# rimelq/VISTAF-RoboSkin-Vision-Integrated-Multimodal-Sensor

Hardware: AMD Instinct MI355X
Metric: frames/sec (224x224 -> force-map) at batch 256 (higher is better)
Workload: dtype f32; 1 GPU; BASELINE configs[2]: batch 256/GPU of 224x224x3 fp16 fringe frames (256 distinct frames) -> 224x224 f32 depth map + force scalars, full FTP path (inpaint, demod, unwrap, detrend, compose, force tail), constants scaled-224; inputs resident in HBM; global_batch=256, input_dtype=fp16, constants=scaled, parallelism=dp1, inflight_batches=3, frames_with_nonzero_status=0

## Files before the change

vistaf-roboskin-vision-integrated-multimodal-sensor_amd/_lib.py:

```python
from __future__ import annotations

import ctypes
import os

_HERE = os.path.dirname(os.path.abspath(__file__))
LIB_PATH = os.path.join(_HERE, "libvistaf_ftp.so")

NSCALARS = 16
NREFINFO = 8
NCONTACT = 16
MAX_CONTACTS = 64
NTRACK = 16
TRACK_NAMES = ["track_id", "age_frames", "parent_row", "events", "overlap_px", "dx", "dy", "dforce_N", "dvolume_cm3", "origin_track_id"]
TRACK_EVENTS = {"born": 1, "split": 2, "merged": 4, "gated": 8}
FATE_ENDED, FATE_NO_ROW = -1, -2 ** 31
NSHAPE = 24
SHAPE_NAMES = ["contact_pixels", "boundary_pixels", "footprint_cx", "footprint_cy", "major_axis_mm", "minor_axis_mm", "orientation_rad",
               "fit_pixels", "fit_status", "apex_x", "apex_y", "apex_depth_mm", "curvature_1_per_mm", "curvature_2_per_mm",
               "curvature_axis_rad", "radius_1_mm", "radius_2_mm", "fit_rms_mm"]
SHAPE_FIT = {"ok": 0, "none": 1, "not_a_cap": 2}
NTAXEL, NTAXELFRAME, TAXEL_NONE = 12, 8, 0xFFFF
TAXEL_NAMES = ["contact_pixels", "contact_area_mm2", "volume_cm3", "mean_depth_mm", "max_depth_mm", "argmax_index", "centroid_x", "centroid_y",
               "force_N", "pressure_kPa"]
TAXEL_FRAME_NAMES = ["active_taxels", "volume_cm3", "force_N", "cop_x", "cop_y", "moment_x_Nmm", "moment_y_Nmm", "peak_taxel"]
# ... 239 lines not shown
MASK_CHAIN_SIGNATURES = {
    "vistaf_ftp_test_mask_chain_fits": (ci, [ci, ci, ci, ci, ci, ci]),
    "vistaf_ftp_test_bad_chain": (ci, [vp, vp, vp, vp, vp, ci, ci, vp, vp, ci, ci, ci, ci, vp]),
    "vistaf_ftp_test_reliable_chain": (ci, [vp, vp, vp, ci, ci, ci, vp, vp, vp, vp, ci, ci, ci, ci, vp]),
    "vistaf_ftp_test_contact_chain": (ci, [vp, vp, vp, vp, cd, cd, ci, ci, vp, vp, vp, vp, ci, ci, ci, ci, vp]),
}
DFT_STAGED_SIGNATURES = {
    "vistaf_ftp_test_dft_forward_v": (ci, [vp, vp, vp, vp, sz, sz, vp, ci, vp, vp, ci, ci, ci, ci, ci, ci, ci, vp]),
    "vistaf_ftp_test_dft_inverse_v": (ci, [vp, ci, vp, vp, sz, sz, vp, vp, vp, vp, vp, sz, vp, vp, vp, ci, ci, ci, ci, ci, ci, vp]),
    "vistaf_ftp_test_dft_staged_fits": (ci, [ci, ci, ci, ci, ci]),
}
GAUSS_STRIP_SIGNATURES = {
    "vistaf_ftp_test_gauss_variant": (ci, [vp, vp, cd, ci, ci, ci, ci, vp]),
    "vistaf_ftp_test_gauss_strip_fits": (ci, [ci, ci, ci]),
}
OUTLINE_SIGNATURES = {
    "vistaf_outline_workspace_bytes": (ci, [ci, ci, ci, ci, P(sz)]),
    "vistaf_outline_measure": (ci, [vp, vp, vp, vp, ci, ci, ci, ci, ci, vp, vp, vp, vp, sz, vp]),
}
TEXTURE_SIGNATURES = {
    "vistaf_texture_workspace_bytes": (ci, [ci, ci, ci, ci, ci, P(sz)]),
    "vistaf_texture_measure": (ci, [vp, vp, vp, vp, vp, cf, cd, ci, ci, cd, cd, ci, ci, ci, ci, vp, vp, vp, vp, sz, vp]),
}
MATCH_SIGNATURES = {
    "vistaf_match_bank_bytes": (ci, [ci, ci, ci, P(i32), P(sz)]),
    "vistaf_match_build_bank": (ci, [P(cf), P(i32), P(i32), ci, ci, ci, cd, vp, sz]),
    "vistaf_match_workspace_bytes": (ci, [ci, ci, ci, ci, ci, ci, ci, P(sz)]),
    "vistaf_match_measure": (ci, [vp, vp, vp, vp, vp, vp, sz, P(i32), cf, ci, ci, cd, cd, ci, ci, ci, ci, vp, vp, vp, vp, sz, vp]),
}
CENTRELINE_SIGNATURES = {
# ... 7 lines not shown
 TEMPORAL_EXPORTS, CLOUD_EXPORTS, MOTION_EXPORTS, PRESSURE_EXPORTS) = (list(group) for group in SIGNATURES.values())

_lib = None


def load():
    global _lib
    if _lib is not None:
        return _lib
    if not os.path.exists(LIB_PATH):
        raise RuntimeError(
            f"{LIB_PATH} is missing: build it with `python __graft_entry__.py` (hipcc --offload-arch=gfx950). "
            "This package has no CPU path."
        )
    lib = ctypes.CDLL(LIB_PATH)
    for group in list(SIGNATURES.values()) + [MASK_CHAIN_SIGNATURES, DFT_STAGED_SIGNATURES, GAUSS_STRIP_SIGNATURES, OUTLINE_SIGNATURES, TEXTURE_SIGNATURES, MATCH_SIGNATURES,
                                                 CENTRELINE_SIGNATURES, CENTRELINE_TEST_SIGNATURES]:
        for name, (restype, argtypes) in group.items():
            fn = getattr(lib, name)
            fn.restype, fn.argtypes = restype, argtypes
    _lib = lib
    return lib


def check(rc: int):
    if rc != 0:
        msg = load().vistaf_ftp_last_error().decode("utf-8", "replace")
        if rc == -1:
            raise ValueError(msg)
        raise RuntimeError(f"vistaf_ftp error {rc}: {msg}")
```

vistaf-roboskin-vision-integrated-multimodal-sensor_amd/csrc/api.hip:

```cpp
#include <hip/hip_runtime.h>
#include <algorithm>
#include <cmath>
#include <cstdio>
#include <cstdlib>
#include <cstring>
#include <map>
#include <string>
#include <vector>

#include "host_util.hpp"
#include "mask_rules.hpp"
#include "mask_bits.hpp"

using namespace vf;
#include "test_hooks.h"
#include "test_hooks_masks.h"
#include "test_hooks_dft.h"
#include "test_hooks_gauss.h"
#ifdef VISTAF_DEBUG
namespace vf { void telea_debug_dump(); void telea_window_debug_dump(int B); void telea_window_mw_debug_dump(int B); void fit_debug_dump(); void unwrap_big_debug_dump(); void unwrap_batch_debug_dump(); }
#endif

static thread_local std::string g_err;
static int fail(int code, const std::string &msg) { g_err = msg; return code; }
namespace vf { int set_error(int code, const std::string &msg) { return fail(code, msg); } }

namespace {

struct GKern { float *d = nullptr; int k = 0; };

enum Stage { ST_GRAY_BAD = 0, ST_INPAINT, ST_PREPROC, ST_DEMOD, ST_RELIABLE, ST_UNWRAP_RANK, ST_UNWRAP, ST_UNWRAP_TREE, ST_DETREND, ST_SMOOTH_FLIP, ST_COMPOSE, ST_MM_BLOB,
             ST_TAIL, ST_COUNT };
const char *kStageNames[ST_COUNT] = {"gray+badpix", "inpaint (k_telea_window_mw)", "illum+blur+apod+median", "pruned-dft demod", "reliable mask",
// ... 32 lines not shown
    std::map<std::string, Named> named;
    DeviceAllocs allocs;
    float *img, *grad, *tmpf, *blurA, *inorm, *iw, *amp, *prod, *quality, *wrapped, *unwrapped, *phase1, *resid0, *detr, *z0, *mplane,
        *num, *den, *hmap, *dist, *z0f, *snum, *unitless, *depth;
    double2 *field, *patch;
    double2 *tmpT;
    uint8_t *bad0, *bad1, *rel0, *rel1, *rel2, *reliable, *contact, *contact_d, *background, *cand, *kept;
    uint8_t *out_rel = nullptr, *hole_cand = nullptr;
    float *hole_med = nullptr, *hole_fill = nullptr;
    int32_t *labels, *area, *rowdist, *parent;
    unsigned int *peak_bits;
    uint16_t *morph_pre;
    void *inpaint_scratch, *inpaint_cl_scratch, *inpaint_win_scratch, *unwrap_scratch;
    void *big_scratch = nullptr;
    size_t big_scratch_bytes = 0;
    int32_t *unwrap_need;
    float *thr_hi, *thr_g, *mu, *amp_thr, *thr3, *thr_used, *bg_med, *core_thr, *core_med, *coef;
    int *cnt_a, *cnt_valid, *rel_count, *contact_count, *bg_count, *bad_count, *flipped;
    unsigned int *gmax;
    int32_t *status;
    int32_t *big_only;
    unsigned long long *cc_best;
    double *scalars;
    float *req_hi, *req_g, *req_med, *req_amp, *req_contact, *req_core, *req_core_med;

    ContactScratch contacts_ws{};
    int last_batch = 0;
    bool last_pairs = false;

    bool timing = false;
// ... 343 lines not shown
    PLANE(unsigned int, peak_bits);
    PLANE(uint16_t, morph_pre);
#undef PLANE
    {
        void *p = nullptr;
        TRY(dalloc(hd, (uint8_t **)&p, inpaint_scratch_bytes(max_batch, h, w))); hd->inpaint_scratch = p;
        TRY(dalloc(hd, (uint8_t **)&p, inpaint_cl_scratch_bytes(max_batch, h, w))); hd->inpaint_cl_scratch = p;
        TRY(dalloc(hd, (uint8_t **)&p, inpaint_win_scratch_bytes(max_batch))); hd->inpaint_win_scratch = p;
        TRY(dalloc(hd, (uint8_t **)&p, unwrap_scratch_bytes(max_batch, h, w))); hd->unwrap_scratch = p;
        if (large_frame((size_t)P)) {
            hd->big_scratch_bytes = big_scratch_bytes(max_batch, h, w);
            TRY(dalloc(hd, (uint8_t **)&p, hd->big_scratch_bytes)); hd->big_scratch = p;
        }
        TRY(dalloc(hd, &hd->unwrap_need, (size_t)max_batch, "unwrap_need", sizeof(int32_t)));
        HIPCHK(hipMemset(hd->unwrap_need, 0xff, (size_t)max_batch * sizeof(int32_t)));
    }
    int pmax = 2 * bwp + 1;
    hd->pmax = pmax;
    TRY(dalloc(hd, &hd->patch, (size_t)max_batch * pmax * pmax, "patch", (size_t)pmax * pmax * sizeof(double2)));
    TRY(dalloc(hd, &hd->tmpT, (size_t)max_batch * (size_t)std::max(h, w) * pmax));
    TRY(dalloc(hd, &hd->Ex, (size_t)w * pmax)); TRY(dalloc(hd, &hd->Gx, (size_t)w * pmax));
    TRY(dalloc(hd, &hd->Ey, (size_t)h * pmax)); TRY(dalloc(hd, &hd->Gy, (size_t)h * pmax));
    TRY(dalloc(hd, &hd->win, (size_t)pmax * pmax)); TRY(dalloc(hd, &hd->geom, 1));
    TRY(dalloc(hd, &hd->cref, (size_t)P)); TRY(dalloc(hd, &hd->amp_ref, (size_t)P));
    hd->named["cref"] = {hd->cref, (size_t)P * sizeof(double2), false}; hd->named["amp_ref"] = {hd->amp_ref, (size_t)P * sizeof(float), false};
    size_t mb = max_batch;
    TRY(dalloc(hd, &hd->thr_hi, mb)); TRY(dalloc(hd, &hd->thr_g, mb)); TRY(dalloc(hd, &hd->mu, mb)); TRY(dalloc(hd, &hd->amp_thr, mb));
    TRY(dalloc(hd, &hd->thr3, mb * 3)); TRY(dalloc(hd, &hd->thr_used, mb)); TRY(dalloc(hd, &hd->bg_med, mb));
    TRY(dalloc(hd, &hd->core_thr, mb)); TRY(dalloc(hd, &hd->core_med, mb)); TRY(dalloc(hd, &hd->coef, mb * 6));
    TRY(dalloc(hd, &hd->cnt_a, mb)); TRY(dalloc(hd, &hd->cnt_valid, mb)); TRY(dalloc(hd, &hd->rel_count, mb));
// ... 121 lines not shown
    const float *qual = hd->quality;
    select(hd, qual, hd->roi, 0, nullptr, false, hd->req_amp, 1, hd->amp_thr, nullptr, B, st);
    {
        const ReliableScratch ws = {hd->rel1, hd->rel2, hd->labels, hd->area, hd->rowdist, hd->dist, hd->cc_best, hd->morph_pre};
        const int tier = reliable_mask_chain(qual, hd->roi, hd->amp_thr, hd->se_close, c.valid_close_iters, c.reliable_edge_margin_px, ws,
                                             hd->tiers.chamfer_twopass != 0, hd->rel0, hd->reliable, hd->rel_count, hd->status,
                                             (hd->tiers.fused_masks & MCH_RELIABLE) != 0, B, h, w, st);
        if (tier < 0) return tier;
    }

    if (timed) hipEventRecord(hd->ev[ST_UNWRAP_RANK], st);
    launch_unwrap(hd->wrapped, qual, hd->reliable, hd->unwrapped, hd->parent, hd->unwrap_scratch, hd->status, B, h, w, st,
                  timed ? hd->ev[ST_UNWRAP_TREE] : nullptr, timed ? hd->ev[ST_UNWRAP] : nullptr, hd->tiers.big_flood_handback != 0, hd->tiers.unwrap_fast ? hd->unwrap_need : nullptr);

    if (timed) hipEventRecord(hd->ev[ST_DETREND], st);
    if (c.plane_order_for_removal > 0)
        launch_robust_polyfit(hd->unwrapped, hd->reliable, c.plane_order_for_removal, c.irls_iters, (float)c.irls_c, 200, 500, hd->coef, hd->phase1, B, h, w, st, chain_scratch(hd));
    else
        HIPCHK(hipMemcpyAsync(hd->phase1, hd->unwrapped, (size_t)B * P * sizeof(float), hipMemcpyDeviceToDevice, st));
    launch_robust_polyfit(hd->phase1, hd->reliable, c.poly_order, c.irls_iters, (float)c.irls_c, 200, 0, hd->coef, hd->resid0, B, h, w, st, chain_scratch(hd));
    select(hd, hd->resid0, hd->reliable, (size_t)P, nullptr, true, hd->req_contact, 3, hd->thr3, nullptr, B, st);
    {
        const ContactScratchPlanes ws = {hd->contact, hd->cand, hd->morph_pre};
        const int tier = contact_mask_chain(hd->resid0, hd->reliable, hd->thr3, hd->rel_count, c.min_contact_frac, c.max_contact_frac, hd->se_contact,
                                            c.dilate_iters, ws, hd->contact_count, hd->thr_used, hd->contact_d, hd->background, hd->bg_count,
                                            (hd->tiers.fused_masks & MCH_CONTACT) != 0, B, h, w, st);
        if (tier < 0) return tier;
    }
    launch_robust_polyfit(hd->phase1, hd->background, c.poly_order, c.irls_iters, (float)c.irls_c, 200, 0, hd->coef, hd->detr, B, h, w, st, chain_scratch(hd));
    select(hd, hd->detr, hd->background, (size_t)P, nullptr, false, hd->req_med, 1, hd->bg_med, nullptr, B, st);

    if (timed) hipEventRecord(hd->ev[ST_SMOOTH_FLIP], st);
    const bool smooth_rel = hd->g_rel.k > 0;
    if (fuses(hd, hd->g_rel)) launch_smooth_reliable(hd->detr, hd->bg_med, hd->reliable, hd->hmap, hd->g_rel.d, hd->g_rel.k, B, h, w, st);
    else if (smooth_rel) {
// ... 213 lines not shown
    const std::string n(name);
    if (n == "inpaint_tier" && value >= 0 && value <= 2) hd->tiers.inpaint = value;
    else if (n == "big_flood_handback") hd->tiers.big_flood_handback = value != 0;
    else if (n == "chamfer_twopass") hd->tiers.chamfer_twopass = value != 0;
    else if (n == "telea_two_tier") hd->tiers.telea_two_tier = value != 0;
    else if (n == "telea_mw") hd->tiers.telea_mw = value != 0;
    else if (n == "big_queue_lds") hd->tiers.big_queue_lds = value != 0;
    else if (n == "big_gq_cap" && (value == 0 || (value >= 64 && (value & (value - 1)) == 0))) hd->tiers.big_gq_cap = value;
    else if (n == "big_fallback") hd->tiers.big_fallback = value != 0;
    else if (n == "unwrap_fast") hd->tiers.unwrap_fast = value != 0;
    else if (n == "big_chain") hd->tiers.big_chain = value != 0;
    else if (n == "select_resident") hd->tiers.select_resident = value != 0;
    else if (n == "dft_staged") hd->tiers.dft_staged = value != 0;
    else if (n == "fused_chains") hd->tiers.fused_chains = value != 0;
    else if (n == "gauss_strip") hd->tiers.gauss_strip = value != 0;
    else if (n == "fused_backend") hd->tiers.fused_backend = value != 0;
    else if (n == "fused_masks" && value >= 0 && value <= 7) hd->tiers.fused_masks = value;
    else if (n == "keep_planes") hd->keep_planes = value != 0;
    else return fail(VISTAF_E_INVALID, "unknown test hook or value: " + n);
    return 0;
}

namespace {
int hook_scratch(int variant, int B, int h, int w, bool chain_ok, void **scratch)
{
    *scratch = nullptr;
    if (variant < 0 || variant > 2) return fail(VISTAF_E_INVALID, "variant must be 0, 1 or 2");
    if (variant == 2 && !chain_ok) return fail(VISTAF_E_INVALID, "variant 2: the k_big.hip chain does not take this batch");
    if (variant == 1 || (variant == 0 && !large_frame((size_t)h * w))) return 0;
    HIPCHK(hipMalloc(scratch, big_scratch_bytes(B, h, w)));
// ... 43 lines not shown
    return rc ? rc : inst;
}

int vistaf_ftp_test_polyfit(const float *z, const uint8_t *mask, int order, int iters, float c, int min_count, int min_mask_count, float *coef,
                            float *resid, int B, int h, int w, int variant, void *stream)
{
    if (!z || !mask || !coef || !resid || B < 1 || h < 1 || w < 1 || (size_t)h * w > 0x7fffffffull || order < 1 || order > 2 || iters < 1)
        return fail(VISTAF_E_INVALID, "bad argument");
    void *scratch = nullptr;
    int rc = hook_scratch(variant, B, h, w, big_frames(B, h * w), &scratch);
    if (rc) return rc;
    const int inst = polyfit_variant(B, h, w, scratch != nullptr);
    launch_robust_polyfit(z, mask, order, iters, c, min_count, min_mask_count, coef, resid, B, h, w, (hipStream_t)stream, scratch);
    rc = hook_finish(scratch, nullptr, (hipStream_t)stream);
    return rc ? rc : inst;
}

int vistaf_ftp_test_gauss_variant(const float *src, float *dst, double sigma, int B, int h, int w, int variant, void *stream)
{
    if (!src || !dst || src == dst || B < 1 || h < 1 || w < 1 || !(sigma > 0)) return fail(VISTAF_E_INVALID, "bad argument");
    if (variant < 0 || variant > 2) return fail(VISTAF_E_INVALID, "variant must be 0, 1 or 2");
    if (gauss_ksize(sigma) > 511) return fail(VISTAF_E_INVALID, "gaussian sigma too large (ksize > 511)");
    const std::vector<float> f = gauss_taps(sigma);
    if (variant == 2 && !gauss_strip_fits(h, w, (int)f.size())) return fail(VISTAF_E_INVALID, "variant 2: the strip kernel does not take this blur");
    float *taps = nullptr, *tmp = nullptr;
    HIPCHK(hipMalloc((void **)&taps, f.size() * sizeof(float)));
    if (hipMalloc((void **)&tmp, (size_t)B * h * w * sizeof(float)) != hipSuccess) { (void)hipFree(taps); return fail(VISTAF_E_HIP, "hipMalloc"); }
    if (hipMemcpy(taps, f.data(), f.size() * sizeof(float), hipMemcpyHostToDevice) != hipSuccess) {
        (void)hipFree(taps); (void)hipFree(tmp);
        return fail(VISTAF_E_HIP, "memcpy taps");
// ... 455 lines not shown
```

vistaf-roboskin-vision-integrated-multimodal-sensor_amd/csrc/k_fit.hip:

```cpp
#include <cstdio>
#include <algorithm>
#include <type_traits>
#include "kernels.hpp"
#ifdef VISTAF_DEBUG
namespace vf { __device__ unsigned long long g_fit_dbg[16]; __device__ unsigned long long g_fit_last; }
#define SEL_STAMP(i) do { if (blockIdx.x == 0 && threadIdx.x == 0) { const unsigned long long t_ = __builtin_amdgcn_s_memtime(); vf::g_fit_dbg[i] += t_ - vf::g_fit_last; vf::g_fit_last = t_; } } while (0)
#define FIT_START() do { if (blockIdx.x == 0 && threadIdx.x == 0) { vf::g_fit_last = __builtin_amdgcn_s_memtime(); vf::g_fit_dbg[10]++; } } while (0)
#else
#define FIT_START() do { } while (0)
#endif
#include "select.hpp"
#include "fit_rules.hpp"
#include "chol.hpp"

namespace vf {

constexpr int FIT_TAB = 4096;
constexpr int FIT_YTAB = 1280;
constexpr int FIT_U = 8;

struct FitCtx {
    const float *z;
    const uint8_t *m;
    const float *tab;
// ... 184 lines not shown
            float xn, yn;
            ctx.coords(p, xn, yn);
            fit = fit_eval(ctx.coef, order, xn, yn);
        }
        out[p] = __fsub_rn(zz, fit);
    }
}

__device__ inline double readlane_f64(double v, int l)
{
    const unsigned long long r = (unsigned long long)__double_as_longlong(v);
    const uint32_t lo = (uint32_t)__builtin_amdgcn_readlane((int)(uint32_t)r, l), hi = (uint32_t)__builtin_amdgcn_readlane((int)(uint32_t)(r >> 32), l);
    return __longlong_as_double((long long)(((unsigned long long)hi << 32) | lo));
}

template <int RP, int NT, int GT>
__device__ __attribute__((always_inline)) inline void robust_polyfit_col_body(const float *__restrict__ z_all, const uint8_t *__restrict__ mask_all, int order,
                                                              int iters, float c, int min_count, int min_mask_count, float *__restrict__ coef_out,
                                                              float *__restrict__ resid_all, int h, int w, int cols_pad, int groups_rt)
{
    static_assert(NT % 64 == 0 && NT >= 256 && NT / 64 <= 16, "block_sum / block_min / block_max scratch holds 16 waves");
    static_assert(RP >= 1 && RP <= 128, "rows per thread live in registers");
    static_assert(GT >= 0 && (GT == 0 || (RP - 1) * GT + GT + 15 < FIT_YTAB), "row table");
    const int groups = GT > 0 ? GT : groups_rt;
    FIT_START();
    __shared__ SelShared sh;
    __shared__ double s_part[NT / 64][21];
    __shared__ float s_coef[6];
    __shared__ float s_yn[FIT_YTAB];
    const size_t b = blockIdx.x;
    const int P = h * w, tid = threadIdx.x, lane = tid & 63, wid = __builtin_amdgcn_readfirstlane(tid >> 6);
    const int nc = order >= 2 ? 6 : 3;
    const float *z = z_all + b * (size_t)P;
    const uint8_t *m = mask_all + b * (size_t)P;
    const float cxf = fit_centre(w), cyf = fit_centre(h);
    for (int i = tid; i < FIT_YTAB; i += NT) s_yn[i] = fit_coord(i, cyf);
    const int col = tid % cols_pad, grp = __builtin_amdgcn_readfirstlane(tid / cols_pad);
    const bool owner = col < w && grp < groups;
    const float xn = fit_coord(col, cxf);
    const float qnan = nanf32();
    float zr[RP];
    uint32_t cntm = 0;
    SelRange rg;
    {
        constexpr int LU = 8;
        uint8_t mk[LU];
#pragma unroll
        for (int u0 = 0; u0 < RP; u0 += LU) {
#pragma unroll
            for (int v = 0; v < LU; v++) {
                const int u = u0 + v;
                if (u < RP) {
                    const int y = grp + groups * u;
                    const bool in = owner && y < h;
                    zr[u] = in ? z[(size_t)y * w + col] : qnan;
                    mk[v] = in ? m[(size_t)y * w + col] : (uint8_t)0;
                }
            }
#pragma unroll
            for (int v = 0; v < LU; v++) {
                const int u = u0 + v;
                if (u < RP) {
                    const float zz = zr[u];
                    const bool ok = mk[v] && finitef(zz);
                    cntm += mk[v] != 0;
                    zr[u] = ok ? zz : qnan;
                    if (ok) rg.add(f2key(zz));
                }
            }
        }
    }
    __syncthreads();
    uint32_t n, zkmin, zkmax;
    rg.reduce(sh.wsum, sh.red64, n, zkmin, zkmax, min_mask_count > 0, cntm);
    __syncthreads();
    const float zmin = key2f(zkmin), zmax = key2f(zkmax);
    const bool do_fit = fit_gate((int)n, (int)cntm, min_count, min_mask_count);
    SEL_STAMP(8);

    float coef[6] = {0.f, 0.f, 0.f, 0.f, 0.f, 0.f};
    float At = 0.f, Bt = 0.f;
    float med = 0.f;
    int mode = 0;
    auto resid_of = [&](int g0, int u, float zz) -> float {
        const float yn = s_yn[g0 + groups * u];
        return __fsub_rn(zz, fit_col_eval(At, Bt, coef[5], yn));
    };
    auto each = [&](auto body) {
        int g0 = grp;
        asm volatile("" : "+s"(g0));
#pragma unroll
        for (int u = 0; u < RP; u++) {
            float r = resid_of(g0, u, zr[u]);
            if (finitef(r)) {
                if (mode) r = fabsf(__fsub_rn(r, med));
                body(f2key(r));
            }
        }
    };

    float csig = 1.f;
    auto irls_step = [&](auto ncc, int it) {
        constexpr int NC = decltype(ncc)::value, DEG = NC == 6 ? 4 : 2;
        constexpr int NM = (DEG + 1) * (DEG + 2) / 2, NV = NM + NC;
        double Pb[5] = {0.0, 0.0, 0.0, 0.0, 0.0}, Qb[3] = {0.0, 0.0, 0.0};
        const float inv_csig = __fdiv_rn(1.0f, csig);
        int g0 = grp;
        asm volatile("" : "+s"(g0));
#pragma unroll
        for (int u = 0; u < RP; u++) {
            const float zz = zr[u];
            if (finitef(__fmul_rn(zz, inv_csig))) {
                float wt = 1.f;
                if (it > 0) {
                    wt = fit_cauchy(resid_of(g0, u, zz), inv_csig);
                }
                const double yd = (double)s_yn[g0 + groups * u];
                const double w2 = (double)wt * (double)wt;
                const double t1 = w2 * yd, t2 = t1 * yd;
                Pb[0] += w2; Pb[1] += t1; Pb[2] += t2;
                const double zw = w2 * (double)zz;
                Qb[0] += zw; Qb[1] = fma(zw, yd, Qb[1]);
                if constexpr (NC == 6) {
// ... 50 lines not shown
        if (nc == 6) irls_step(std::integral_constant<int, 6>(), it);
        else irls_step(std::integral_constant<int, 3>(), it);
        if (it == iters - 1) break;
        mode = 0;
        const FitKeys kr = fit_resid_range(coef, zmin, zmax);
        const float medr = block_median_each<NT>(each, sh, n, kr.kmin, kr.kmax);
        __syncthreads();
        med = medr; mode = 1;
        const FitKeys ka = fit_mad_range(kr, medr);
        const float mad = block_median_each<NT>(each, sh, n, ka.kmin, ka.kmax);
        __syncthreads();
        mode = 0;
        csig = fit_csig(c, mad);
    }
    if (tid < 6) coef_out[b * 6 + tid] = do_fit ? coef[tid] : 0.f;
    float *out = resid_all + b * (size_t)P;
    if (owner) {
#pragma unroll
        for (int u = 0; u < RP; u++) {
            const int y = grp + groups * u;
            if (y < h && !finitef(zr[u])) zr[u] = z[(size_t)y * w + col];
        }
#pragma unroll
        for (int u = 0; u < RP; u++) {
            const int y = grp + groups * u;
            if (y < h) {
                const float fit = do_fit ? fit_eval(coef, order, xn, s_yn[y]) : 0.f;
                out[(size_t)y * w + col] = __fsub_rn(zr[u], fit);
            }
        }
    }
    SEL_STAMP(9);
}

#ifdef VISTAF_DEBUG
void fit_debug_dump()
{
    unsigned long long d[16];
    if (hipMemcpyFromSymbol(d, HIP_SYMBOL(g_fit_dbg), sizeof(d)) != hipSuccess) return;
    printf("[fit dbg] frame 0, %llu launches so far, cycle sums: load %llu | column sums %llu | reduce+solve %llu | hist clear %llu | hist pass %llu | bucket search %llu | "
           "collect %llu | sort %llu | second statistic pass %llu | residual plane %llu || of reduce+solve: wave sums %llu | partials %llu | solve %llu | rest in [reduce+solve]\n", d[10], d[8], d[6], d[7], d[0], d[1], d[2], d[3], d[4], d[5], d[9], d[11], d[12], d[13]);
}
#endif

#define VF_FIT_ARGS const float *__restrict__ z_all, const uint8_t *__restrict__ mask_all, int order, int iters, float c, int min_count, int min_mask_count, \
                    float *__restrict__ coef_out, float *__restrict__ resid_all, int h, int w, int cols_pad, int groups
#define VF_FIT_PASS z_all, mask_all, order, iters, c, min_count, min_mask_count, coef_out, resid_all, h, w, cols_pad, groups
template <int RP, int GT>
__global__ __launch_bounds__(SEL_T) void k_robust_polyfit_col(VF_FIT_ARGS) { robust_polyfit_col_body<RP, SEL_T, GT>(VF_FIT_PASS); }
#undef VF_FIT_ARGS
#undef VF_FIT_PASS

int polyfit_variant(int B, int h, int w, bool big, int *cols_pad_out, int *groups_out)
{
    if (big && big_frames(B, h * w)) return FITV_BIG;
    constexpr int NT = SEL_T;
    const int cols_pad = ((w + 63) / 64) * 64;
    const int groups = cols_pad <= NT ? std::min(NT / cols_pad, h) : 0;
    const int need = groups ? (h + groups - 1) / groups : 1 << 30;
    if (cols_pad_out) *cols_pad_out = cols_pad;
    if (groups_out) *groups_out = groups;
    if (need <= 64 && h + groups * 16 <= FIT_YTAB) {
        if (groups == 4 && need > 32) return need <= 48 ? FITV_COL48_G4 : need <= 56 ? FITV_COL56_G4 : FITV_COL64_G4;
        return need <= 16 ? FITV_COL16 : need <= 32 ? FITV_COL32 : need <= 48 ? FITV_COL48 : need <= 56 ? FITV_COL56 : FITV_COL64;
// ... 18 lines not shown
    case FITV_COL32: VF_FIT_COL((k_robust_polyfit_col<32, 0>), SEL_T, groups); break;
    case FITV_COL48: VF_FIT_COL((k_robust_polyfit_col<48, 0>), SEL_T, groups); break;
    case FITV_COL56: VF_FIT_COL((k_robust_polyfit_col<56, 0>), SEL_T, groups); break;
    case FITV_COL64: VF_FIT_COL((k_robust_polyfit_col<64, 0>), SEL_T, groups); break;
    case FITV_GENERIC:
        hipLaunchKernelGGL(k_robust_polyfit, dim3(B), dim3(SEL_T), 0, st, z, mask, order, iters, c, min_count, min_mask_count, coef_out, resid_out, h, w,
                           (uint32_t)(0x100000000ull / (unsigned)w) + 1u);
        break;
    default:
        hipLaunchKernelGGL(k_robust_polyfit, dim3(B), dim3(SEL_T), 0, st, z, mask, order, iters, c, min_count, min_mask_count, coef_out, resid_out, h, w, 0u);
        break;
    }
#undef VF_FIT_COL
}

}
```

vistaf-roboskin-vision-integrated-multimodal-sensor_amd/csrc/kernels.hpp:

```cpp
#pragma once
#include <hip/hip_runtime.h>
#include <stdint.h>
#include <vector>
#include "common.hpp"

namespace vf {

struct Tiers {
    int inpaint = 2;
    int big_flood_handback = 0;
    int chamfer_twopass = 0;
    int telea_two_tier = 1;
    int unwrap_fast = 1;
    int big_chain = 1;
    int big_queue_lds = 1;
    int big_gq_cap = 0;
    int big_fallback = 1;
    int telea_mw = 1;
    int fused_backend = 1;
    int select_resident = 1;
    int fused_masks = 7;
    int dft_staged = 1;
    int fused_chains = 1;
    int gauss_strip = 1;
};

inline bool large_frame(size_t P) { return P >= 262144; }

struct ScratchLayout;
struct ScratchRegion;
using ScratchRec = std::vector<ScratchRegion>;

struct RowSpanSE {
    int k;
    int8_t lo[33];
    int8_t hi[33];
};

void launch_to_gray(const void *frames, int format, float *gray, int B, int P, hipStream_t st, int w = 0);
// ... 116 lines not shown
void launch_inpaint_big_handback(int32_t *status, int32_t *only, int B, hipStream_t st);
void launch_inpaint_clusters(float *img, const uint8_t *bad, int range, void *scratch, uint8_t **bad_big_out, ClusterPlanes *left, int B, int h, int w,
                             hipStream_t st);

bool unwrap_fast_supported(int h, int w);
size_t unwrap_scratch_bytes(int B, int h, int w, ScratchRec *rec = nullptr);
enum UnwrapTier { UWT_RANK16 = 0, UWT_BITMAP = 1, UWT_GENERIC = 2 };
int unwrap_tier(int h, int w, bool big_handback = false);
void launch_unwrap(const float *wrapped, const float *quality, const uint8_t *mask, float *unwrapped, int32_t *parent,
                   void *scratch, int32_t *status, int B, int h, int w, hipStream_t st, hipEvent_t ev_mid,
                   hipEvent_t ev_flood = nullptr, bool big_handback = false, int32_t *need_buf = nullptr);

void launch_robust_polyfit(const float *z, const uint8_t *mask, int order, int iters, float c, int min_count, int min_mask_count, float *coef_out,
                           float *resid_out, int B, int h, int w, hipStream_t st, void *big_scratch = nullptr);
enum FitVariant { FITV_BIG = 0, FITV_GENERIC, FITV_GENERIC_DIV, FITV_COL16, FITV_COL32, FITV_COL48, FITV_COL56, FITV_COL64, FITV_COL48_G4, FITV_COL56_G4,
                  FITV_COL64_G4, FITV_COUNT };
int polyfit_variant(int B, int h, int w, bool big, int *cols_pad_out = nullptr, int *groups_out = nullptr);

void launch_zeroed_keep_nan(const float *detr, const float *bg_med, const uint8_t *reliable, float *hmap, int B, int P, hipStream_t st);
void launch_hole_candidates(const float *hmap, const uint8_t *reliable, const float *dist, int ksize, float frac_thr, float min_dist, uint8_t *cand,
                            int B, int h, int w, hipStream_t st);
void launch_hole_tmp(const float *hmap, const uint8_t *reliable, const uint8_t *cand, const float *med, float *tmp, int B, int P, hipStream_t st);
void launch_hole_zin(float *tmp_zin, const float *fill, int B, int P, hipStream_t st);
void launch_hole_merge(float *hmap, const uint8_t *reliable, const uint8_t *cand, const float *zin, uint8_t *out_rel, int B, int P, hipStream_t st);

constexpr int LAB_SHIFT = 12, LAB_SHIFT2 = 15, LAB_GAMMA_SHIFT = 3, LAB_CBRT_N = 256 * 3 / 2 * (1 << LAB_GAMMA_SHIFT);
struct LabCoef { int c[9]; int lscale, lshift; };
void launch_feature_planes(const uint8_t *bgr, const uint16_t *gamma_tab, const uint16_t *cbrt_tab, const LabCoef &cf, bool blur, float *L, float *a,
                           float *b, float *gray, int H, int W, hipStream_t st);
void launch_color_support(const float *a, const float *b, const uint8_t *light_d, const uint8_t *roi_eff, const uint8_t *sat, float chroma_min,
                          float *chroma, uint8_t *support, size_t n, hipStream_t st);

// ... 94 lines not shown
```

Baseline: 78370 frames/s.

## Fuse chained detrend polyfits and add a row-window register variant with retry

The two sequential robust polyfits (plane removal, then poly detrend) now run as a two-pass chain inside one kernel, with the residual of the first pass kept in registers as input to the second. A windowed variant also holds fewer rows per thread by loading only the span of rows that contain mask pixels. Frames whose mask span exceeds that window set a need flag, and a retry kernel with the full row count then processes only those frames. The aim is to cut a kernel launch and a full-plane reread, and to lower register pressure. The cost is an extra mask scan, a second launch for the retry, and more template instances.

```diff
diff --git a/vistaf-roboskin-vision-integrated-multimodal-sensor_amd/_lib.py b/vistaf-roboskin-vision-integrated-multimodal-sensor_amd/_lib.py
--- a/vistaf-roboskin-vision-integrated-multimodal-sensor_amd/_lib.py
+++ b/vistaf-roboskin-vision-integrated-multimodal-sensor_amd/_lib.py
@@ -277,6 +277,11 @@
     "vistaf_ftp_test_gauss_variant": (ci, [vp, vp, cd, ci, ci, ci, ci, vp]),
     "vistaf_ftp_test_gauss_strip_fits": (ci, [ci, ci, ci]),
 }
+FIT_WINDOW_SIGNATURES = {
+    "vistaf_ftp_test_polyfit_window": (ci, [vp, vp, ci, ci, cf, ci, ci, vp, vp, ci, ci, ci, ci, vp, vp]),
+    "vistaf_ftp_test_polyfit_chain": (ci, [vp, vp, ci, ci, ci, cf, ci, ci, ci, vp, vp, vp, ci, ci, ci, ci, vp, vp]),
+    "vistaf_ftp_test_polyfit_window_instance": (ci, [ci, ci, ci]),
+}
 OUTLINE_SIGNATURES = {
     "vistaf_outline_workspace_bytes": (ci, [ci, ci, ci, ci, P(sz)]),
     "vistaf_outline_measure": (ci, [vp, vp, vp, vp, ci, ci, ci, ci, ci, vp, vp, vp, vp, sz, vp]),
@@ -314,7 +319,8 @@
             "This package has no CPU path."
         )
     lib = ctypes.CDLL(LIB_PATH)
-    for group in list(SIGNATURES.values()) + [MASK_CHAIN_SIGNATURES, DFT_STAGED_SIGNATURES, GAUSS_STRIP_SIGNATURES, OUTLINE_SIGNATURES, TEXTURE_SIGNATURES, MATCH_SIGNATURES,
+    for group in list(SIGNATURES.values()) + [MASK_CHAIN_SIGNATURES, DFT_STAGED_SIGNATURES, GAUSS_STRIP_SIGNATURES, FIT_WINDOW_SIGNATURES, OUTLINE_SIGNATURES, TEXTURE_SIGNATURES,
+                                                 MATCH_SIGNATURES,
                                                  CENTRELINE_SIGNATURES, CENTRELINE_TEST_SIGNATURES]:
         for name, (restype, argtypes) in group.items():
             fn = getattr(lib, name)
diff --git a/vistaf-roboskin-vision-integrated-multimodal-sensor_amd/csrc/api.hip b/vistaf-roboskin-vision-integrated-multimodal-sensor_amd/csrc/api.hip
--- a/vistaf-roboskin-vision-integrated-multimodal-sensor_amd/csrc/api.hip
+++ b/vistaf-roboskin-vision-integrated-multimodal-sensor_amd/csrc/api.hip
@@ -17,6 +17,7 @@
 #include "test_hooks_masks.h"
 #include "test_hooks_dft.h"
 #include "test_hooks_gauss.h"
+#include "test_hooks_fit.h"
 #ifdef VISTAF_DEBUG
 namespace vf { void telea_debug_dump(); void telea_window_debug_dump(int B); void telea_window_mw_debug_dump(int B); void fit_debug_dump(); void unwrap_big_debug_dump(); void unwrap_batch_debug_dump(); }
 #endif
@@ -79,6 +80,7 @@
     void *inpaint_scratch, *inpaint_cl_scratch, *inpaint_win_scratch, *unwrap_scratch;
     void *big_scratch = nullptr;
     size_t big_scratch_bytes = 0;
+    int32_t *fit_need;
     int32_t *unwrap_need;
     float *thr_hi, *thr_g, *mu, *amp_thr, *thr3, *thr_used, *bg_med, *core_thr, *core_med, *coef;
     int *cnt_a, *cnt_valid, *rel_count, *contact_count, *bg_count, *bad_count, *flipped;
@@ -452,6 +454,8 @@
         }
         TRY(dalloc(hd, &hd->unwrap_need, (size_t)max_batch, "unwrap_need", sizeof(int32_t)));
         HIPCHK(hipMemset(hd->unwrap_need, 0xff, (size_t)max_batch * sizeof(int32_t)));
+        TRY(dalloc(hd, &hd->fit_need, (size_t)max_batch, "fit_need", sizeof(int32_t)));
+        HIPCHK(hipMemset(hd->fit_need, 0xff, (size_t)max_batch * sizeof(int32_t)));
     }
     int pmax = 2 * bwp + 1;
     hd->pmax = pmax;
@@ -603,11 +607,15 @@
                   timed ? hd->ev[ST_UNWRAP_TREE] : nullptr, timed ? hd->ev[ST_UNWRAP] : nullptr, hd->tiers.big_flood_handback != 0, hd->tiers.unwrap_fast ? hd->unwrap_need : nullptr);
 
     if (timed) hipEventRecord(hd->ev[ST_DETREND], st);
-    if (c.plane_order_for_removal > 0)
-        launch_robust_polyfit(hd->unwrapped, hd->reliable, c.plane_order_for_removal, c.irls_iters, (float)c.irls_c, 200, 500, hd->coef, hd->phase1, B, h, w, st, chain_scratch(hd));
-    else
+    const bool fit_win = hd->tiers.fit_window != 0;
+    if (c.plane_order_for_removal > 0) {
+        const FitSecond detrend1 = {c.poly_order, 0, hd->resid0};
+        launch_robust_polyfit_window(hd->unwrapped, hd->reliable, c.plane_order_for_removal, c.irls_iters, (float)c.irls_c, 200, 500, hd->coef, hd->phase1, &detrend1,
+                                     hd->fit_need, fit_win, 0, B, h, w, st, chain_scratch(hd));
+    } else {
         HIPCHK(hipMemcpyAsync(hd->phase1, hd->unwrapped, (size_t)B * P * sizeof(float), hipMemcpyDeviceToDevice, st));
-    launch_robust_polyfit(hd->phase1, hd->reliable, c.poly_order, c.irls_iters, (float)c.irls_c, 200, 0, hd->coef, hd->resid0, B, h, w, st, chain_scratch(hd));
+        launch_robust_polyfit(hd->phase1, hd->reliable, c.poly_order, c.irls_iters, (float)c.irls_c, 200, 0, hd->coef, hd->resid0, B, h, w, st, chain_scratch(hd));
+    }
     select(hd, hd->resid0, hd->reliable, (size_t)P, nullptr, true, hd->req_contact, 3, hd->thr3, nullptr, B, st);
     {
         const ContactScratchPlanes ws = {hd->contact, hd->cand, hd->morph_pre};
@@ -851,6 +859,7 @@
     else if (n == "dft_staged") hd->tiers.dft_staged = value != 0;
     else if (n == "fused_chains") hd->tiers.fused_chains = value != 0;
     else if (n == "gauss_strip") hd->tiers.gauss_strip = value != 0;
+    else if (n == "fit_window") hd->tiers.fit_window = value != 0;
     else if (n == "fused_backend") hd->tiers.fused_backend = value != 0;
     else if (n == "fused_masks" && value >= 0 && value <= 7) hd->tiers.fused_masks = value;
     else if (n == "keep_planes") hd->keep_planes = value != 0;
@@ -924,6 +933,47 @@
     launch_robust_polyfit(z, mask, order, iters, c, min_count, min_mask_count, coef, resid, B, h, w, (hipStream_t)stream, scratch);
     rc = hook_finish(scratch, nullptr, (hipStream_t)stream);
     return rc ? rc : inst;
+}
+
+static int fit_window_hook(const float *z, const uint8_t *mask, int order, int iters, float c, int min_count, int min_mask_count, float *coef, float *resid,
+                           const FitSecond *second, int B, int h, int w, int variant, int32_t *need_out, void *stream)
+{
+    if (!z || !mask || !coef || !resid || (second && !second->resid_out) || B < 1 || h < 1 || w < 1 || (size_t)h * w > 0x7fffffffull || order < 1 || order > 2 ||
+        (second && (second->order < 1 || second->order > 2)) || iters < 1)
+        return fail(VISTAF_E_INVALID, "bad argument");
+    if (variant < 0 || variant > 2) return fail(VISTAF_E_INVALID, "variant must be 0, 1 or 2");
+    void *scratch = nullptr;
+    int rc = hook_scratch(0, B, h, w, big_frames(B, h * w), &scratch);
+    if (rc) return rc;
+    const bool has_window = polyfit_window_variant(B, h, w, scratch != nullptr) >= 0;
+    if (variant == 1 && !has_window) { if (scratch) (void)hipFree(scratch); return fail(VISTAF_E_INVALID, "variant 1: no window instance for this frame size"); }
+    int32_t *need = nullptr;
+    if (hipMalloc((void **)&need, (size_t)B * sizeof(int32_t)) != hipSuccess) { if (scratch) (void)hipFree(scratch); return fail(VISTAF_E_HIP, "hipMalloc"); }
+    hipError_t e = hipMemsetAsync(need, 0xff, (size_t)B * sizeof(int32_t), (hipStream_t)stream);
+    const int inst = launch_robust_polyfit_window(z, mask, order, iters, c, min_count, min_mask_count, coef, resid, second, need, Tiers().fit_window != 0, variant,
+                                                  B, h, w, (hipStream_t)stream, scratch);
+    if (e == hipSuccess && need_out) e = hipMemcpyAsync(need_out, need, (size_t)B * sizeof(int32_t), hipMemcpyDeviceToDevice, (hipStream_t)stream);
+    rc = hook_finish(scratch, need, (hipStream_t)stream);
+    if (!rc && e != hipSuccess) rc = fail(VISTAF_E_HIP, std::string("need: ") + hipGetErrorString(e));
+    return rc ? rc : inst;
+}
+int vistaf_ftp_test_polyfit_window(const float *z, const uint8_t *mask, int order, int iters, float c, int min_count, int min_mask_count, float *coef,
+                                   float *resid, int B, int h, int w, int variant, int32_t *need_out, void *stream)
+{
+    return fit_window_hook(z, mask, order, iters, c, min_count, min_mask_count, coef, resid, nullptr, B, h, w, variant, need_out, stream);
+}
+int vistaf_ftp_test_polyfit_chain(const float *z, const uint8_t *mask, int order1, int order2, int iters, float c, int min_count, int min_mask_count1,
+                                  int min_mask_count2, float *coef, float *resid1, float *resid2, int B, int h, int w, int variant, int32_t *need_out, void *stream)
+{
+    const FitSecond second = {order2, min_mask_count2, resid2};
+    return fit_window_hook(z, mask, order1, iters, c, min_count, min_mask_count1, coef, resid1, &second, B, h, w, variant, need_out, stream);
+}
+int vistaf_ftp_test_polyfit_window_instance(int B, int h, int w)
+{
+    if (B < 1 || h < 1 || w < 1 || (size_t)h * w > 0x7fffffffull) return fail(VISTAF_E_INVALID, "bad argument");
+    const bool big = large_frame((size_t)h * w);
+    const int plain = polyfit_variant(B, h, w, big), win = polyfit_window_variant(B, h, w, big);
+    return win >= 0 ? win : plain;
 }
 
 int vistaf_ftp_test_gauss_variant(const float *src, float *dst, double sigma, int B, int h, int w, int variant, void *stream)
diff --git a/vistaf-roboskin-vision-integrated-multimodal-sensor_amd/csrc/k_fit.hip b/vistaf-roboskin-vision-integrated-multimodal-sensor_amd/csrc/k_fit.hip
--- a/vistaf-roboskin-vision-integrated-multimodal-sensor_amd/csrc/k_fit.hip
+++ b/vistaf-roboskin-vision-integrated-multimodal-sensor_amd/csrc/k_fit.hip
@@ -222,10 +222,18 @@
     return __longlong_as_double((long long)(((unsigned long long)hi << 32) | lo));
 }
 
-template <int RP, int NT, int GT>
+struct FitChain {
+    int *need_flag;
+    int npass;
+    int order2, min_mask_count2;
+    float *resid2_all;
+};
+constexpr int fit_plain_rp(int rp) { return rp == 16 ? 32 : rp == 32 ? 48 : rp == 48 ? 56 : 64; }
+template <int RP, int NT, int GT, bool WIN = false, bool PASSES = false>
 __device__ __attribute__((always_inline)) inline void robust_polyfit_col_body(const float *__restrict__ z_all, const uint8_t *__restrict__ mask_all, int order,
                                                               int iters, float c, int min_count, int min_mask_count, float *__restrict__ coef_out,
-                                                              float *__restrict__ resid_all, int h, int w, int cols_pad, int groups_rt)
+                                                              float *__restrict__ resid_all, int h, int w, int cols_pad, int groups_rt,
+                                                              const FitChain ex = FitChain())
 {
     static_assert(NT % 64 == 0 && NT >= 256 && NT / 64 <= 16, "block_sum / block_min / block_max scratch holds 16 waves");
     static_assert(RP >= 1 && RP <= 128, "rows per thread live in registers");
@@ -238,9 +246,12 @@
     __shared__ float s_yn[FIT_YTAB];
     const size_t b = blockIdx.x;
     const int P = h * w, tid = threadIdx.x, lane = tid & 63, wid = __builtin_amdgcn_readfirstlane(tid >> 6);
-    const int nc = order >= 2 ? 6 : 3;
+    int nc = order >= 2 ? 6 : 3;
     const float *z = z_all + b * (size_t)P;
     const uint8_t *m = mask_all + b * (size_t)P;
+    if constexpr (PASSES && !WIN) {
+        if (ex.need_flag && ex.need_flag[b] == 0) return;
+    }
     const float cxf = fit_centre(w), cyf = fit_centre(h);
     for (int i = tid; i < FIT_YTAB; i += NT) s_yn[i] = fit_coord(i, cyf);
     const int col = tid % cols_pad, grp = __builtin_amdgcn_readfirstlane(tid / cols_pad);
@@ -250,7 +261,62 @@
     float zr[RP];
     uint32_t cntm = 0;
     SelRange rg;
-    {
+    unsigned long long mbits = 0;
+    int u0 = 0, y0 = grp;
+    const uint32_t gw = (uint32_t)(groups * w);
+    const int need = (h + groups - 1) / groups;
+    if constexpr (WIN) {
+        constexpr int RPF = fit_plain_rp(RP), MU = 16;
+        static_assert(RPF <= 64, "one bit per slot");
+        const uint32_t mo = (uint32_t)(grp * w + col);
+#pragma unroll
+        for (int a = 0; a < RPF; a += MU) {
+            uint8_t mk[MU];
+#pragma unroll
+            for (int v = 0; v < MU; v++) {
+                const int u = a + v;
+                if (u < RPF) mk[v] = (owner && grp + groups * u < h) ? m[mo + (uint32_t)u * gw] : (uint8_t)0;
+            }
+#pragma unroll
+            for (int v = 0; v < MU; v++) {
+                const int u = a + v;
+                if (u < RPF) mbits |= (unsigned long long)(mk[v] != 0) << u;
+            }
+        }
+        const int first = mbits ? __builtin_ctzll(mbits) : 0, last = mbits ? 63 - __builtin_clzll(mbits) : -1;
+        const int over = __syncthreads_or(last - first + 1 > RP);
+        if (tid == 0) ex.need_flag[b] = over ? 1 : 0;
+        if (over) return;
+        u0 = max(0, min(first, need - RP));
+        y0 = grp + groups * u0;
+        mbits >>= u0;
+    }
+    const uint32_t o0 = (uint32_t)(y0 * w + col);
+    if constexpr (WIN || PASSES) {
+        constexpr int LU = 8;
+#pragma unroll
+        for (int a = 0; a < RP; a += LU) {
+            uint8_t mk[LU];
+#pragma unroll
+            for (int v = 0; v < LU; v++) {
+                const int u = a + v;
+                if (u < RP) {
+                    const bool in = owner && y0 + groups * u < h;
+                    zr[u] = in ? z[o0 + (uint32_t)u * gw] : qnan;
+                    if constexpr (!WIN) mk[v] = in ? m[o0 + (uint32_t)u * gw] : (uint8_t)0;
+                }
+            }
+            if constexpr (!WIN) {
+#pragma unroll
+                for (int v = 0; v < LU; v++) {
+                    const int u = a + v;
+                    if (u < RP) mbits |= (unsigned long long)(mk[v] != 0) << u;
+                }
+            }
+        }
+#pragma unroll
+        for (int u = 0; u < RP; u++) zr[u] = (mbits >> u & 1) ? zr[u] : qnan;
+    } else {
         constexpr int LU = 8;
         uint8_t mk[LU];
 #pragma unroll
@@ -276,6 +342,24 @@
                     if (ok) rg.add(f2key(zz));
                 }
             }
+        }
+    }
+    const int npass = PASSES ? ex.npass : 1;
+    const float *zsrc = z;
+    float *out = nullptr;
+#pragma unroll 1
+    for (int pass = 0;; pass++) {
+    if constexpr (PASSES) {
+        if (pass) { order = ex.order2; nc = order >= 2 ? 6 : 3; min_mask_count = ex.min_mask_count2; zsrc = out; out = ex.resid2_all + b * (size_t)P; }
+        else out = resid_all + b * (size_t)P;
+        cntm = (uint32_t)__builtin_popcountll(mbits);
+        rg = SelRange();
+#pragma unroll
+        for (int u = 0; u < RP; u++) {
+            const float zz = zr[u];
+            const bool ok = finitef(zz);
+            zr[u] = ok ? zz : qnan;
+            if (ok) rg.add(f2key(zz));
         }
     }
     __syncthreads();
@@ -295,8 +379,9 @@
         return __fsub_rn(zz, fit_col_eval(At, Bt, coef[5], yn));
     };
     auto each = [&](auto body) {
-        int g0 = grp;
-        asm volatile("" : "+s"(g0));
+        int g0 = y0;
+        if constexpr (WIN) asm volatile("" : "+v"(g0));
+        else asm volatile("" : "+s"(g0));
 #pragma unroll
         for (int u = 0; u < RP; u++) {
             float r = resid_of(g0, u, zr[u]);
@@ -313,8 +398,9 @@
         constexpr int NM = (DEG + 1) * (DEG + 2) / 2, NV = NM + NC;
         double Pb[5] = {0.0, 0.0, 0.0, 0.0, 0.0}, Qb[3] = {0.0, 0.0, 0.0};
         const float inv_csig = __fdiv_rn(1.0f, csig);
-        int g0 = grp;
-        asm volatile("" : "+s"(g0));
+        int g0 = y0;
+        if constexpr (WIN) asm volatile("" : "+v"(g0));
+        else asm volatile("" : "+s"(g0));
 #pragma unroll
         for (int u = 0; u < RP; u++) {
             const float zz = zr[u];
@@ -395,7 +481,48 @@
         csig = fit_csig(c, mad);
     }
     if (tid < 6) coef_out[b * 6 + tid] = do_fit ? coef[tid] : 0.f;
-    float *out = resid_all + b * (size_t)P;
+    if constexpr (!PASSES) out = resid_all + b * (size_t)P;
+    if constexpr (WIN || PASSES) {
+        if (owner) {
+            unsigned long long mb = mbits;
+            uint32_t oo = o0, gg = gw;
+            int yy = y0;
+            asm volatile("" : "+v"(mb), "+v"(oo), "+s"(gg), "+v"(yy));
+#pragma unroll
+            for (int u = 0; u < RP; u++) {
+                if (yy + groups * u < h && !finitef(zr[u])) zr[u] = zsrc[oo + (uint32_t)u * gg];
+            }
+#pragma unroll
+            for (int u = 0; u < RP; u++) {
+                const int y = yy + groups * u;
+                if (y < h) {
+                    const float fit = do_fit ? fit_eval(coef, order, xn, s_yn[y]) : 0.f;
+                    const float o = __fsub_rn(zr[u], fit);
+                    out[oo + (uint32_t)u * gg] = o;
+                    if constexpr (PASSES) zr[u] = (mb >> u & 1) ? o : qnan;
+                }
+            }
+            if constexpr (WIN) {
+                constexpr int NO = fit_plain_rp(RP) - RP;
+                float zo[NO];
+                int yo[NO];
+#pragma unroll
+                for (int j = 0; j < NO; j++) {
+                    int s = u0 + RP + j;
+                    if (s >= need) s -= need;
+                    yo[j] = (j < need - RP && grp + groups * s < h) ? grp + groups * s : -1;
+                    zo[j] = yo[j] >= 0 ? zsrc[(uint32_t)(yo[j] * w + col)] : 0.f;
+                }
+#pragma unroll
+                for (int j = 0; j < NO; j++) {
+                    if (yo[j] >= 0) {
+                        const float fit = do_fit ? fit_eval(coef, order, xn, s_yn[yo[j]]) : 0.f;
+                        out[(uint32_t)(yo[j] * w + col)] = __fsub_rn(zo[j], fit);
+                    }
+                }
+            }
+        }
+    } else {
     if (owner) {
 #pragma unroll
         for (int u = 0; u < RP; u++) {
@@ -411,7 +538,11 @@
             }
         }
     }
+    }
     SEL_STAMP(9);
+    if constexpr (!PASSES) break;
+    else if (pass + 1 >= npass) break;
+    }
 }
 
 #ifdef VISTAF_DEBUG
@@ -429,6 +560,14 @@
 #define VF_FIT_PASS z_all, mask_all, order, iters, c, min_count, min_mask_count, coef_out, resid_all, h, w, cols_pad, groups
 template <int RP, int GT>
 __global__ __launch_bounds__(SEL_T) void k_robust_polyfit_col(VF_FIT_ARGS) { robust_polyfit_col_body<RP, SEL_T, GT>(VF_FIT_PASS); }
+#define VF_FIT_CHAIN_ARGS int order2, int min_mask_count2, float *resid2_all, int npass, int *need_flag
+#define VF_FIT_CHAIN_PASS FitChain{need_flag, npass, order2, min_mask_count2, resid2_all}
+template <int RP, int GT>
+__global__ __launch_bounds__(SEL_T) void k_robust_polyfit_colwin(VF_FIT_ARGS, VF_FIT_CHAIN_ARGS) { robust_polyfit_col_body<RP, SEL_T, GT, true, true>(VF_FIT_PASS, VF_FIT_CHAIN_PASS); }
+template <int RP, int GT>
+__global__ __launch_bounds__(SEL_T) void k_robust_polyfit_col_retry(VF_FIT_ARGS, VF_FIT_CHAIN_ARGS) { robust_polyfit_col_body<RP, SEL_T, GT, false, true>(VF_FIT_PASS, VF_FIT_CHAIN_PASS); }
+#undef VF_FIT_CHAIN_ARGS
+#undef VF_FIT_CHAIN_PASS
 #undef VF_FIT_ARGS
 #undef VF_FIT_PASS
 
@@ -477,4 +616,65 @@
 #undef VF_FIT_COL
 }
 
-}
+int polyfit_window_of(int plain_variant)
+{
+    switch (plain_variant) {
+    case FITV_COL32: return FITV_WIN16;
+    case FITV_COL48: return FITV_WIN32;
+    case FITV_COL56: return FITV_WIN48;
+    case FITV_COL64: return FITV_WIN56;
+    case FITV_COL48_G4: return FITV_WIN32_G4;
+    case FITV_COL56_G4: return FITV_WIN48_G4;
+    case FITV_COL64_G4: return FITV_WIN56_G4;
+    default: return -1;
+    }
+}
+int polyfit_window_variant(int B, int h, int w, bool big) { return polyfit_window_of(polyfit_variant(B, h, w, big)); }
+
+namespace {
+using FitChainKernel = void (*)(const float *, const uint8_t *, int, int, float, int, int, float *, float *, int, int, int, int, int, int, float *, int, int *);
+struct FitWindowKernels { FitChainKernel win, retry; int gt; };
+FitWindowKernels fit_window_kernels(int plain_variant)
+{
+    switch (plain_variant) {
+    case FITV_COL16: return {nullptr, k_robust_polyfit_col_retry<16, 0>, 0};
+    case FITV_COL32: return {k_robust_polyfit_colwin<16, 0>, k_robust_polyfit_col_retry<32, 0>, 0};
+    case FITV_COL48: return {k_robust_polyfit_colwin<32, 0>, k_robust_polyfit_col_retry<48, 0>, 0};
+    case FITV_COL56: return {k_robust_polyfit_colwin<48, 0>, k_robust_polyfit_col_retry<56, 0>, 0};
+    case FITV_COL64: return {k_robust_polyfit_colwin<56, 0>, k_robust_polyfit_col_retry<64, 0>, 0};
+    case FITV_COL48_G4: return {k_robust_polyfit_colwin<32, 4>, k_robust_polyfit_col_retry<48, 4>, 4};
+    case FITV_COL56_G4: return {k_robust_polyfit_colwin<48, 4>, k_robust_polyfit_col_retry<56, 4>, 4};
+    case FITV_COL64_G4: return {k_robust_polyfit_colwin<56, 4>, k_robust_polyfit_col_retry<64, 4>, 4};
+    default: return {nullptr, nullptr, 0};
+    }
+}
+}
+
+int launch_robust_polyfit_window(const float *z, const uint8_t *mask, int order, int iters, float c, int min_count, int min_mask_count, float *coef_out,
+                                 float *resid_out, const FitSecond *second, int *need_flag, bool window, int force, int B, int h, int w, hipStream_t st,
+                                 void *big_scratch)
+{
+    int cols_pad = 0, groups = 0;
+    const int variant = polyfit_variant(B, h, w, big_scratch != nullptr, &cols_pad, &groups);
+    const FitWindowKernels k = fit_window_kernels(variant);
+    if (force == FIT_PLAIN || (force == 0 && (!window || !k.retry))) {
+        launch_robust_polyfit(z, mask, order, iters, c, min_count, min_mask_count, coef_out, resid_out, B, h, w, st, big_scratch);
+        if (second) launch_robust_polyfit(resid_out, mask, second->order, iters, c, min_count, second->min_mask_count, coef_out, second->resid_out, B, h, w, st, big_scratch);
+        return variant;
+    }
+    const int gr = k.gt ? k.gt : groups;
+    const int order2 = second ? second->order : order, mmc2 = second ? second->min_mask_count : 0, npass = second ? 2 : 1;
+    float *resid2 = second ? second->resid_out : nullptr;
+#define VF_FIT_CHAIN(KERNEL, NEED) hipLaunchKernelGGL(KERNEL, dim3(B), dim3(SEL_T), 0, st, z, mask, order, iters, c, min_count, min_mask_count, coef_out, resid_out, h, w, cols_pad, gr, \
+                                                      order2, mmc2, resid2, npass, NEED)
+    if (!k.win) {
+        VF_FIT_CHAIN(k.retry, (int *)nullptr);
+        return variant;
+    }
+    VF_FIT_CHAIN(k.win, need_flag);
+    if (force != FIT_WINDOW_ONLY) VF_FIT_CHAIN(k.retry, need_flag);
+#undef VF_FIT_CHAIN
+    return polyfit_window_of(variant);
+}
+
+}
diff --git a/vistaf-roboskin-vision-integrated-multimodal-sensor_amd/csrc/kernels.hpp b/vistaf-roboskin-vision-integrated-multimodal-sensor_amd/csrc/kernels.hpp
--- a/vistaf-roboskin-vision-integrated-multimodal-sensor_amd/csrc/kernels.hpp
+++ b/vistaf-roboskin-vision-integrated-multimodal-sensor_amd/csrc/kernels.hpp
@@ -23,6 +23,7 @@
     int dft_staged = 1;
     int fused_chains = 1;
     int gauss_strip = 1;
+    int fit_window = 1;
 };
 
 inline bool large_frame(size_t P) { return P >= 262144; }
@@ -169,8 +170,14 @@
 void launch_robust_polyfit(const float *z, const uint8_t *mask, int order, int iters, float c, int min_count, int min_mask_count, float *coef_out,
                            float *resid_out, int B, int h, int w, hipStream_t st, void *big_scratch = nullptr);
 enum FitVariant { FITV_BIG = 0, FITV_GENERIC, FITV_GENERIC_DIV, FITV_COL16, FITV_COL32, FITV_COL48, FITV_COL56, FITV_COL64, FITV_COL48_G4, FITV_COL56_G4,
-                  FITV_COL64_G4, FITV_COUNT };
+                  FITV_COL64_G4, FITV_WIN16, FITV_WIN32, FITV_WIN48, FITV_WIN56, FITV_WIN32_G4, FITV_WIN48_G4, FITV_WIN56_G4, FITV_COUNT };
 int polyfit_variant(int B, int h, int w, bool big, int *cols_pad_out = nullptr, int *groups_out = nullptr);
+int polyfit_window_variant(int B, int h, int w, bool big);
+struct FitSecond { int order, min_mask_count; float *resid_out; };
+enum FitForce { FIT_WINDOW_ONLY = 1, FIT_PLAIN = 2 };
+int launch_robust_polyfit_window(const float *z, const uint8_t *mask, int order, int iters, float c, int min_count, int min_mask_count, float *coef_out,
+                                 float *resid_out, const FitSecond *second, int *need_flag, bool window, int force, int B, int h, int w, hipStream_t st,
+                                 void *big_scratch);
 
 void launch_zeroed_keep_nan(const float *detr, const float *bg_med, const uint8_t *reliable, float *hmap, int B, int P, hipStream_t st);
 void launch_hole_candidates(const float *hmap, const uint8_t *reliable, const float *dist, int ksize, float frac_thr, float min_dist, uint8_t *cand,
```

New measurement: 79310 frames/s, median of 6. 1.2% higher.
